# saltoricristiano/lidog

Hardware: AMD Instinct MI355X
Metric: LiDAR scans/sec, MinkUNet34+BEV training step @120k pts (higher is better)
Workload: dtype f32

## Files before the change

### lidog_amd/csrc/conv2d.h

```cpp
#pragma once
#include "common.h"

typedef float f32x16 __attribute__((ext_vector_type(16)));

#define IG_T 128
#define IG_LD 132

struct IgParams {
    const float *A;
    const float *Bm;
    float *D;
    int Bn, Cin, H, W, Cout, Ho, Wo;
    int Mi, Nj, Kd;
    int py, px, nky, nkx, Hc, Wc;
    int ky0, kystep, kx0, kxstep;
    int k_chunk;
};

enum { IG_FWD = 0, IG_DGRAD = 1, IG_WGRAD = 2 };

struct IgClasses {
    IgParams c[4];
    int first[5];
    int n;
    int row_tiles[4];
    long long list_off[4];
};

#define C2_KB 32

void lidog_launch_repack_dgrad_all(const float *W, int Cin, int Cout, float *Wd, hipStream_t st);
```

### lidog_amd/csrc/conv2d.hip

```cpp
#include "common.h"
#include "clock_stamp.h"

#include "conv2d.h"

#define WG_KB 32
#define WG_LD 129
__global__ __launch_bounds__(256) void k_conv_wgrad(IgParams p) {
    __shared__ float As[WG_KB * WG_LD];
    __shared__ float Bs[WG_KB * WG_LD];
    const int tid = threadIdx.x, lane = tid & 63, wave = tid >> 6;
    const int i0 = blockIdx.y * IG_T, j0 = blockIdx.x * IG_T;
    const int HoWo = p.Ho * p.Wo, HW = p.H * p.W;
    const int k_begin = blockIdx.z * p.k_chunk;
    const int k_end = k_begin + p.k_chunk < p.Kd ? k_begin + p.k_chunk : p.Kd;
    const int kk = tid & 31, rg = tid >> 5;

    int cpk[16];
    unsigned a_mask = 0;
#pragma unroll
    for (int r = 0; r < 16; ++r) {
        int j = j0 + rg + 8 * r;
        cpk[r] = -1;
        if (j < p.Nj) {
            int ci = j / 9, t = j - ci * 9;
// ... 76 lines not shown
        load_stage();
        float af[2], bf[2], an[2], bn[2];
        af[0] = a_rd[0]; af[1] = a_rd[32];
        bf[0] = b_rd[0]; bf[1] = b_rd[32];
#pragma unroll
        for (int k2 = 0; k2 < WG_KB / 2; ++k2) {
            if (k2 + 1 < WG_KB / 2) {
                an[0] = a_rd[(2 * k2 + 2) * WG_LD]; an[1] = a_rd[(2 * k2 + 2) * WG_LD + 32];
                bn[0] = b_rd[(2 * k2 + 2) * WG_LD]; bn[1] = b_rd[(2 * k2 + 2) * WG_LD + 32];
            }
            __builtin_amdgcn_sched_barrier(0);
            acc[0][0] = __builtin_amdgcn_mfma_f32_32x32x2f32(af[0], bf[0], acc[0][0], 0, 0, 0);
            acc[0][1] = __builtin_amdgcn_mfma_f32_32x32x2f32(af[0], bf[1], acc[0][1], 0, 0, 0);
            acc[1][0] = __builtin_amdgcn_mfma_f32_32x32x2f32(af[1], bf[0], acc[1][0], 0, 0, 0);
            acc[1][1] = __builtin_amdgcn_mfma_f32_32x32x2f32(af[1], bf[1], acc[1][1], 0, 0, 0);
            __builtin_amdgcn_sched_barrier(0);
            if (k2 + 1 < WG_KB / 2) {
                af[0] = an[0]; af[1] = an[1];
                bf[0] = bn[0]; bf[1] = bn[1];
            }
        }
    }

#pragma unroll
    for (int tj = 0; tj < 2; ++tj) {
        int j = j0 + wj + 32 * tj + li;
        if (j >= p.Nj) continue;
        float *d = p.D + (size_t)blockIdx.z * p.Mi * p.Nj + j;
#pragma unroll
        for (int ti = 0; ti < 2; ++ti) {
#pragma unroll
            for (int e = 0; e < 16; ++e) {
                int i = i0 + wi + 32 * ti + (e & 3) + 8 * (e >> 2) + 4 * kh;
                if (i < p.Mi) d[(size_t)i * p.Nj] = acc[ti][tj][e];
            }
        }
    }
}

template <int MODE, int WM, int TI, int TJ>
__device__ __forceinline__ void conv_s2_tile(const IgParams &p, const int bx, const int by, float *__restrict__ As,
                                             float *__restrict__ Bs) {
    constexpr int TMR = WM * TI * 32;
    constexpr int AV = (TMR * C2_KB / 4) / 256;
    static_assert((4 / WM) * TJ * 32 == IG_T, "tile is 128 pixels wide");
    static_assert((TMR * C2_KB / 4) % 256 == 0, "A stage must divide over the threads");
    extern __shared__ int2 s_tab[];
    const int tid = threadIdx.x, lane = tid & 63, wave = tid >> 6;
    const int i0 = by * TMR, j0 = bx * IG_T;
    const int HoWo = p.Ho * p.Wo, HW = p.H * p.W;
    const int kw = __builtin_amdgcn_readfirstlane(tid >> 7);
    const int nt = p.nky * p.nkx;

    for (int kk = tid; kk < p.Kd; kk += 256) {
        int koff, t;
        if (MODE == IG_FWD) {
            int ci = kk / 9;
            t = kk - ci * 9;
            int ty = t / 3, tx = t - ty * 3;
            koff = ci * HW + (ty - 1) * p.W + (tx - 1);
        } else {
            int co = kk / nt, tap = kk - co * nt;
            int ty = tap / p.nkx, tx = tap - ty * p.nkx;
            koff = co * HoWo - ty * p.Wo - tx;
            t = ty * 2 + tx;
        }
        s_tab[kk] = make_int2(koff, t);
    }

    const int j = j0 + (tid & 127);
    const bool jvalid = j < p.Nj;
    const int jj = jvalid ? j : 0;
    int base, safe;
    unsigned tapmask = 0;
    if (MODE == IG_FWD) {
        int pb = jj / HoWo, r = jj - pb * HoWo;
        int yo = r / p.Wo, xo = r - yo * p.Wo;
        base = pb * p.Cin * HW + (2 * yo) * p.W + 2 * xo;
        safe = base;
#pragma unroll
        for (int ty = 0; ty < 3; ++ty)
#pragma unroll
            for (int tx = 0; tx < 3; ++tx) {
                int y = 2 * yo - 1 + ty, x = 2 * xo - 1 + tx;
                tapmask |= (unsigned)(y >= 0 && y < p.H && x >= 0 && x < p.W) << (ty * 3 + tx);
            }
    } else {
        int hw = p.Hc * p.Wc;
        int pb = jj / hw, r = jj - pb * hw;
        int pyy = (r / p.Wc) * 2 + p.py, pxx = (r % p.Wc) * 2 + p.px;
        int y0 = (pyy + 1 - p.ky0) >> 1, x0 = (pxx + 1 - p.kx0) >> 1;
        safe = pb * p.Cout * HoWo;
        base = safe + y0 * p.Wo + x0;
#pragma unroll
        for (int ty = 0; ty < 2; ++ty)
#pragma unroll
            for (int tx = 0; tx < 2; ++tx)
                tapmask |= (unsigned)(y0 - ty >= 0 && y0 - ty < p.Ho && x0 - tx >= 0 && x0 - tx < p.Wo)
                           << (ty * 2 + tx);
    }
    if (!jvalid) tapmask = 0;

    const float *a_ptr[AV];
    bool a_ok[AV];
#pragma unroll
    for (int v = 0; v < AV; ++v) {
        int f = tid + 256 * v;
        int i = i0 + (f >> 3);
        a_ok[v] = i < p.Mi;
        a_ptr[v] = p.A + (size_t)(a_ok[v] ? i : p.Mi - 1) * p.Kd + (f & 7) * 4;
    }
    __syncthreads();

    float4 ra[AV];
    float rb[16];
    unsigned okbits = 0;
    auto load_stage = [&](int k0) {
#pragma unroll
        for (int v = 0; v < AV; ++v) ra[v] = *reinterpret_cast<const float4 *>(a_ptr[v] + k0);
        okbits = 0;
#pragma unroll
        for (int r = 0; r < 16; ++r) {
            const int2 e = s_tab[k0 + kw + 2 * r];
            const unsigned ok = (tapmask >> e.y) & 1u;
            okbits |= ok << r;
            rb[r] = p.Bm[ok ? base + e.x : safe];
        }
    };
    auto store_stage = [&]() {
#pragma unroll
        for (int v = 0; v < AV; ++v) {
            int f = tid + 256 * v;
            int il = f >> 3, q = f & 7;
            const bool ok = a_ok[v];
            As[(q * 4 + 0) * IG_LD + il] = ok ? ra[v].x : 0.f;
            As[(q * 4 + 1) * IG_LD + il] = ok ? ra[v].y : 0.f;
            As[(q * 4 + 2) * IG_LD + il] = ok ? ra[v].z : 0.f;
            As[(q * 4 + 3) * IG_LD + il] = ok ? ra[v].w : 0.f;
        }
#pragma unroll
        for (int r = 0; r < 16; ++r) Bs[(kw + 2 * r) * IG_LD + (tid & 127)] = ((okbits >> r) & 1u) ? rb[r] : 0.f;
    };

    f32x16 acc[TI][TJ];
#pragma unroll
    for (int a = 0; a < TI; ++a)
#pragma unroll
        for (int b = 0; b < TJ; ++b)
#pragma unroll
            for (int e = 0; e < 16; ++e) acc[a][b][e] = 0.f;
    const int wi = (WM == 1 ? 0 : (wave >> 1)) * (TI * 32), wj = (WM == 1 ? wave : (wave & 1)) * (TJ * 32);
    const int li = lane & 31, kh = lane >> 5;
    const float *a_rd = &As[kh * IG_LD + wi + li];
    const float *b_rd = &Bs[kh * IG_LD + wj + li];

    load_stage(0);
    for (int k0 = 0; k0 < p.Kd; k0 += C2_KB) {
        __syncthreads();
        store_stage();
        __syncthreads();
        load_stage(k0 + C2_KB < p.Kd ? k0 + C2_KB : k0);
        float af[TI], bf[TJ], an[TI], bn[TJ];
#pragma unroll
        for (int a = 0; a < TI; ++a) af[a] = a_rd[32 * a];
#pragma unroll
        for (int b = 0; b < TJ; ++b) bf[b] = b_rd[32 * b];
#pragma unroll
        for (int k2 = 0; k2 < C2_KB / 2; ++k2) {
            if (k2 + 1 < C2_KB / 2) {
#pragma unroll
                for (int a = 0; a < TI; ++a) an[a] = a_rd[(2 * k2 + 2) * IG_LD + 32 * a];
#pragma unroll
                for (int b = 0; b < TJ; ++b) bn[b] = b_rd[(2 * k2 + 2) * IG_LD + 32 * b];
            }
            __builtin_amdgcn_sched_barrier(0);
#pragma unroll
            for (int a = 0; a < TI; ++a)
#pragma unroll
                for (int b = 0; b < TJ; ++b)
                    acc[a][b] = __builtin_amdgcn_mfma_f32_32x32x2f32(af[a], bf[b], acc[a][b], 0, 0, 0);
            __builtin_amdgcn_sched_barrier(0);
            if (k2 + 1 < C2_KB / 2) {
#pragma unroll
                for (int a = 0; a < TI; ++a) af[a] = an[a];
#pragma unroll
                for (int b = 0; b < TJ; ++b) bf[b] = bn[b];
            }
        }
    }

#pragma unroll
    for (int tj = 0; tj < TJ; ++tj) {
        int jo = j0 + wj + 32 * tj + li;
        if (jo >= p.Nj) continue;
        size_t col_off, i_stride;
        if (MODE == IG_FWD) {
            int b = jo / HoWo;
            col_off = (size_t)b * p.Cout * HoWo + (jo - b * HoWo);
            i_stride = HoWo;
        } else {
            int hw = p.Hc * p.Wc;
            int b = jo / hw, r = jo - b * hw;
            int y = (r / p.Wc) * 2 + p.py, x = (r % p.Wc) * 2 + p.px;
            col_off = (size_t)b * p.Cin * HW + (size_t)y * p.W + x;
            i_stride = HW;
        }
#pragma unroll
        for (int ti = 0; ti < TI; ++ti) {
#pragma unroll
            for (int e = 0; e < 16; ++e) {
                int i = i0 + wi + 32 * ti + (e & 3) + 8 * (e >> 2) + 4 * kh;
                if (i < p.Mi) p.D[col_off + (size_t)i * i_stride] = acc[ti][tj][e];
            }
        }
    }
}

template <int MODE, int WM, int TI, int TJ>
__global__ __launch_bounds__(256) void k_conv_s2(IgClasses pc) {
    __shared__ float As[C2_KB * IG_LD];
    __shared__ float Bs[C2_KB * IG_LD];
    const int x = blockIdx.x;
    int cls = 0;
    while (cls + 1 < pc.n && x >= pc.first[cls + 1]) ++cls;
    const IgParams p = pc.c[cls];
    const int r = x - pc.first[cls];
    const int rt = pc.row_tiles[cls];
    LIDOG_STAMP_BEGIN()
    conv_s2_tile<MODE, WM, TI, TJ>(p, r / rt, r % rt, As, Bs);
    LIDOG_STAMP_END()
}

__global__ __launch_bounds__(256) void k_repack_dgrad_all(const float *__restrict__ W, int Cin, int Cout,
                                                          float *__restrict__ Wd) {
    const int64_t cc = (int64_t)Cin * Cout;
    int64_t e = (int64_t)blockIdx.x * 256 + threadIdx.x;
    if (e >= 9 * cc) return;
    const int cls = e < cc ? 0 : e < 3 * cc ? 1 : e < 5 * cc ? 2 : 3;
    const int64_t base = cls == 0 ? 0 : cls == 1 ? cc : cls == 2 ? 3 * cc : 5 * cc;
    const int py = cls >> 1, px = cls & 1;
    const int nky = py ? 2 : 1, nkx = px ? 2 : 1, ky0 = py ? 0 : 1, kx0 = px ? 0 : 1, nt = nky * nkx;
    const int64_t l = e - base;
    int kd = (int)(l % ((int64_t)Cout * nt));
    int ci = (int)(l / ((int64_t)Cout * nt));
    int co = kd / nt, tap = kd % nt;
    int ky = ky0 + (tap / nkx) * 2, kx = kx0 + (tap % nkx) * 2;
    Wd[e] = W[(((size_t)co * Cin + ci) * 3 + ky) * 3 + kx];
}

void lidog_launch_repack_dgrad_all(const float *W, int Cin, int Cout, float *Wd, hipStream_t st) {
    const int64_t total = 9 * (int64_t)Cin * Cout;
    k_repack_dgrad_all<<<(unsigned)cdiv64(total, 256), 256, 0, st>>>(W, Cin, Cout, Wd);
}

__global__ __launch_bounds__(256) void k_sum_splits(const float *__restrict__ partial, int64_t n, int splits,
                                                    int64_t stride, float *__restrict__ out) {
    int64_t i = (int64_t)blockIdx.x * 256 + threadIdx.x;
    if (i >= n) return;
    float acc = partial[i];
    for (int s = 1; s < splits; ++s) acc += partial[(size_t)s * stride + i];
    out[i] = acc;
}

#define PW_MAXCO 8
__global__ __launch_bounds__(256) void k_pw_fwd(const float *__restrict__ X, const float *__restrict__ W,
                                                const float *__restrict__ bias, int Cin, int Cout, int64_t HW,
                                                int64_t total, float *__restrict__ Y) {
    int64_t e = (int64_t)blockIdx.x * 256 + threadIdx.x;
    if (e >= total) return;
    int64_t b = e / HW, pix = e - b * HW;
    float acc[PW_MAXCO];
#pragma unroll
    for (int co = 0; co < PW_MAXCO; ++co) acc[co] = 0.f;
    const float *x = X + (size_t)b * Cin * HW + pix;
// ... 64 lines not shown
            dst[Cout * Cin + co] = (float)(red[PW_MAXCO + co][0] + red[PW_MAXCO + co][1] + red[PW_MAXCO + co][2] +
                                           red[PW_MAXCO + co][3]);
    }
}

static int out_dim(int H, int k, int s, int p) { return (H + 2 * p - k) / s + 1; }

extern "C" int lidog_conv2d_fwd(const float *x, const float *w, const float *bias, int32_t B, int32_t Cin, int32_t H,
                                int32_t W, int32_t Cout, int32_t ksize, int32_t stride, int32_t pad, float *y,
                                void *stream) {
    hipStream_t st = (hipStream_t)stream;
    if (ksize == 1) {
        LIDOG_REQUIRE(stride == 1 && pad == 0 && Cout <= PW_MAXCO, "conv2d_fwd: 1x1 path needs stride 1, Cout <= 8");
        int64_t HW = (int64_t)H * W, total = (int64_t)B * HW;
        if (total) k_pw_fwd<<<(unsigned)cdiv64(total, 256), 256, 0, st>>>(x, w, bias, Cin, Cout, HW, total, y);
        LIDOG_LAUNCH_CHECK();
        return 0;
    }
    LIDOG_REQUIRE(ksize == 3 && stride == 2 && pad == 1 && bias == nullptr,
                  "conv2d_fwd: MFMA path implements k3 s2 p1 without bias (Encoder2D)");
    LIDOG_REQUIRE((Cin * 9) % C2_KB == 0, "conv2d_fwd: Cin*9 must be a multiple of 32");
    IgParams p = {};
    p.A = w; p.Bm = x; p.D = y;
    p.Bn = B; p.Cin = Cin; p.H = H; p.W = W; p.Cout = Cout;
    p.Ho = out_dim(H, 3, 2, 1); p.Wo = out_dim(W, 3, 2, 1);
    p.Mi = Cout; p.Nj = B * p.Ho * p.Wo; p.Kd = Cin * 9;
    if (p.Nj == 0) return 0;
    LIDOG_REQUIRE((int64_t)B * Cin * H * W < ((int64_t)1 << 31) && (int64_t)p.Kd * 8 <= 24576,
                  "conv2d_fwd: tensor too large for 32-bit offsets / reduction table");
    IgClasses pc = {};
    pc.c[0] = p;
    pc.n = 1;
    pc.row_tiles[0] = (int)cdiv64(p.Mi, IG_T);
    pc.first[1] = (int)cdiv64(p.Nj, IG_T) * pc.row_tiles[0];
    k_conv_s2<IG_FWD, 2, 2, 2><<<(unsigned)pc.first[pc.n], 256, (size_t)p.Kd * sizeof(int2), st>>>(pc);
    LIDOG_LAUNCH_CHECK();
    return 0;
}

extern "C" int lidog_conv2d_dgrad(const float *gy, const float *w, int32_t B, int32_t Cin, int32_t H, int32_t W,
                                  int32_t Cout, int32_t ksize, int32_t stride, int32_t pad, float *gx, float *ws,
                                  void *stream) {
    hipStream_t st = (hipStream_t)stream;
    if (ksize == 1) {
        LIDOG_REQUIRE(stride == 1 && pad == 0 && Cout <= PW_MAXCO, "conv2d_dgrad: 1x1 path needs stride 1, Cout <= 8");
        int64_t HW = (int64_t)H * W, total = (int64_t)B * HW;
        if (total) k_pw_dgrad<<<(unsigned)cdiv64(total, 256), 256, 0, st>>>(gy, w, Cin, Cout, HW, total, gx);
        LIDOG_LAUNCH_CHECK();
        return 0;
    }
    LIDOG_REQUIRE(ksize == 3 && stride == 2 && pad == 1, "conv2d_dgrad: MFMA path implements k3 s2 p1");
    LIDOG_REQUIRE(ws != nullptr, "conv2d_dgrad: needs a 9*Cin*Cout float workspace for the repacked weights");
    LIDOG_REQUIRE(Cout % C2_KB == 0, "conv2d_dgrad: Cout must be a multiple of 32");
    LIDOG_REQUIRE((int64_t)B * Cout * out_dim(H, 3, 2, 1) * out_dim(W, 3, 2, 1) < ((int64_t)1 << 31) &&
                      (int64_t)Cout * 4 * 8 <= 24576,
                  "conv2d_dgrad: tensor too large for 32-bit offsets / reduction table");
    int Ho = out_dim(H, 3, 2, 1), Wo = out_dim(W, 3, 2, 1);
    float *slab = ws;
    lidog_launch_repack_dgrad_all(w, Cin, Cout, ws, st);
    const bool rows96 = Cin % 128 != 0 && Cin % 96 == 0;
    IgClasses pc = {};
    IgParams cls_p[4];
    for (int py = 0; py < 2; ++py) {
        for (int px = 0; px < 2; ++px) {
            IgParams &p = cls_p[2 * py + px];
            p = IgParams{};
            p.Bm = gy; p.D = gx;
            p.Bn = B; p.Cin = Cin; p.H = H; p.W = W; p.Cout = Cout; p.Ho = Ho; p.Wo = Wo;
            p.py = py; p.px = px;
            p.nky = py ? 2 : 1; p.ky0 = py ? 0 : 1; p.kystep = 2;
            p.nkx = px ? 2 : 1; p.kx0 = px ? 0 : 1; p.kxstep = 2;
            p.Hc = (H - py + 1) / 2; p.Wc = (W - px + 1) / 2;
            int nt = p.nky * p.nkx;
            p.Mi = Cin; p.Nj = B * p.Hc * p.Wc; p.Kd = Cout * nt;
            int64_t total = (int64_t)Cin * Cout * nt;
            p.A = slab;
            slab += total;
        }
    }
    const int rt = rows96 ? Cin / 96 : (int)cdiv64(Cin, IG_T);
    size_t tab = 0;
    for (int cls : {3, 1, 2, 0}) {
        const IgParams &p = cls_p[cls];
        if (p.Nj <= 0) continue;
        pc.c[pc.n] = p;
        pc.row_tiles[pc.n] = rt;
        pc.first[pc.n + 1] = pc.first[pc.n] + (int)cdiv64(p.Nj, IG_T) * rt;
        ++pc.n;
        if ((size_t)p.Kd * sizeof(int2) > tab) tab = (size_t)p.Kd * sizeof(int2);
    }
    if (pc.n > 0) {
        if (rows96) k_conv_s2<IG_DGRAD, 1, 3, 1><<<(unsigned)pc.first[pc.n], 256, tab, st>>>(pc);
        else k_conv_s2<IG_DGRAD, 2, 2, 2><<<(unsigned)pc.first[pc.n], 256, tab, st>>>(pc);
    }
    LIDOG_LAUNCH_CHECK();
    return 0;
}

extern "C" int lidog_conv2d_wgrad(const float *x, const float *gy, int32_t B, int32_t Cin, int32_t H, int32_t W,
                                  int32_t Cout, int32_t ksize, int32_t stride, int32_t pad, float *gw, float *gbias,
                                  float *ws, int64_t ws_floats, void *stream) {
    hipStream_t st = (hipStream_t)stream;
    if (ksize == 1) {
        LIDOG_REQUIRE(stride == 1 && pad == 0 && Cout <= PW_MAXCO, "conv2d_wgrad: 1x1 path needs stride 1, Cout <= 8");
        const int splits = B * PW_QUARTERS;
        const int64_t slab = (int64_t)Cout * Cin + Cout;
        LIDOG_REQUIRE(ws != nullptr && ws_floats >= splits * slab,
                      "conv2d_wgrad: 1x1 path needs a workspace of %lld floats", (long long)(splits * slab));
        LIDOG_REQUIRE((int64_t)H * W < ((int64_t)1 << 31), "conv2d_wgrad: image too large");
        if (B == 0 || H * W == 0) return 0;
        k_pw_wgrad<<<dim3((unsigned)Cin, (unsigned)splits), 256, 0, st>>>(x, gy, Cin, Cout, H * W, ws);
        k_sum_splits<<<(unsigned)cdiv64((int64_t)Cout * Cin, 256), 256, 0, st>>>(ws, (int64_t)Cout * Cin, splits, slab, gw);
        if (gbias) k_sum_splits<<<1, 256, 0, st>>>(ws + (int64_t)Cout * Cin, Cout, splits, slab, gbias);
        LIDOG_LAUNCH_CHECK();
        return 0;
    }
    LIDOG_REQUIRE(ksize == 3 && stride == 2 && pad == 1 && gbias == nullptr, "conv2d_wgrad: MFMA path implements k3 s2 p1");
    IgParams p = {};
    p.A = gy; p.Bm = x;
    p.Bn = B; p.Cin = Cin; p.H = H; p.W = W; p.Cout = Cout;
    p.Ho = out_dim(H, 3, 2, 1); p.Wo = out_dim(W, 3, 2, 1);
    p.Mi = Cout; p.Nj = Cin * 9; p.Kd = B * p.Ho * p.Wo;
    int64_t slab = (int64_t)p.Mi * p.Nj;
    int tiles = (int)(cdiv64(p.Nj, IG_T) * cdiv64(p.Mi, IG_T));
    int splits = 1024 / tiles;
    if (splits < 1) splits = 1;
    LIDOG_REQUIRE(Cout % 8 == 0, "conv2d_wgrad: Cout must be a multiple of 8");
    LIDOG_REQUIRE((int64_t)Cin * H * W < ((int64_t)1 << 27) && (int64_t)B * Cin * H * W < ((int64_t)1 << 31) &&
                      (int64_t)B * Cout * p.Ho * p.Wo < ((int64_t)1 << 31),
                  "conv2d_wgrad: tensor too large for the packed 32-bit offsets");
    int64_t max_by_k = cdiv64(p.Kd, 4 * WG_KB);
    if (splits > max_by_k) splits = (int)(max_by_k < 1 ? 1 : max_by_k);
    if ((int64_t)splits * slab > ws_floats) splits = (int)(ws_floats / slab);
    LIDOG_REQUIRE(splits >= 1, "conv2d_wgrad: workspace too small (%lld floats needed per split)", (long long)slab);
    p.k_chunk = (int)(cdiv64(cdiv64(p.Kd, splits), WG_KB) * WG_KB);
    splits = (int)cdiv64(p.Kd, p.k_chunk);
    p.D = (splits == 1) ? gw : ws;
    dim3 grid((unsigned)cdiv64(p.Nj, IG_T), (unsigned)cdiv64(p.Mi, IG_T), (unsigned)splits);
    k_conv_wgrad<<<grid, 256, 0, st>>>(p);
    if (splits > 1) k_sum_splits<<<(unsigned)cdiv64(slab, 256), 256, 0, st>>>(ws, slab, splits, slab, gw);
    LIDOG_LAUNCH_CHECK();
    return 0;
}

__global__ __launch_bounds__(256) void k_adam(float *__restrict__ p, const float *__restrict__ g,
                                              float *__restrict__ m, float *__restrict__ v, int64_t n, float lr_bc1,
// ... 29 lines not shown
```

### lidog_amd/csrc/conv2d_sparse.hip

```cpp
#include <vector>

#include "conv2d.h"

__global__ __launch_bounds__(256) void k_support_rowbits(const int32_t *__restrict__ sup, int64_t rows, int W,
                                                         int words, uint64_t *__restrict__ bits) {
    const int64_t row = (int64_t)blockIdx.x * 4 + (threadIdx.x >> 6);
    const int lane = threadIdx.x & 63;
    if (row >= rows) return;
    const int32_t *s = sup + row * W;
    for (int w = 0; w < words; ++w) {
        const int x = w * 64 + lane;
        const bool v = x < W && s[x] >= 0;
        const uint64_t bal = __ballot(v);
        if (lane == 0) bits[row * words + w] = bal;
    }
}

struct ListGeom {
    int C, H, W, Hc, Wc, Nj;
    int ya, ny, xlo, xhi;
    uint64_t mask;
};

__device__ __forceinline__ void tile_list(const uint64_t *__restrict__ bits, int words, const ListGeom &g,
// ... 106 lines not shown
    off += 4 * (int64_t)L.fwd_tiles;
    L.groups = (C + WA_GC - 1) / WA_GC;
    L.glists_off = off;
    off += (int64_t)L.groups * (L.fwd_tiles + 1);
    for (int cls = 0; cls < 4; ++cls) {
        int py = cls >> 1, px = cls & 1;
        int Hc = (H - py + 1) / 2, Wc = (W - px + 1) / 2;
        L.dgrad_tiles[cls] = (int)cdiv64((int64_t)B * Hc * Wc, IG_T);
        L.dgrad_off[cls] = off;
        off += (int64_t)L.dgrad_tiles[cls] * (C + 1);
    }
    L.total = off;
    return L;
}

extern "C" int64_t lidog_conv2d_support_ws(int32_t B, int32_t Cin, int32_t H, int32_t W) {
    return act_layout(B, Cin, H, W).total;
}

extern "C" int lidog_conv2d_support(const int32_t *support, int32_t B, int32_t Cin, int32_t H, int32_t W,
                                    int32_t *act, void *stream) {
    hipStream_t st = (hipStream_t)stream;
    LIDOG_REQUIRE(Cin >= 1 && Cin <= 128, "conv2d_support: 1 <= Cin <= 128");
    LIDOG_REQUIRE((int64_t)B * Cin * H * W < ((int64_t)1 << 31), "conv2d_support: tensor too large");
    if ((int64_t)B * H * W == 0) return 0;
    ActLayout L = act_layout(B, Cin, H, W);
    uint64_t *bits = reinterpret_cast<uint64_t *>(act + L.bits_off);
    int64_t rows = (int64_t)B * Cin * H;
    if (support)
        k_support_rowbits<<<(unsigned)cdiv64(rows, 4), 256, 0, st>>>(support, rows, W, L.words, bits);
    ListGeom g;
    g.C = Cin; g.H = H; g.W = W;
    g.Hc = out_dim2(H); g.Wc = out_dim2(W); g.Nj = B * g.Hc * g.Wc;
    g.ya = -1; g.ny = 3; g.xlo = -1; g.xhi = 1; g.mask = ~0ull;
    uint64_t *tbits = reinterpret_cast<uint64_t *>(act + L.tbits_off);
    k_tile_lists<<<(unsigned)L.fwd_tiles, 128, 0, st>>>(bits, L.words, g, act + L.fwd_off, tbits);
    k_group_lists<<<(unsigned)L.groups, 256, 0, st>>>(tbits, L.fwd_tiles, Cin, act + L.glists_off);
    ListGeom4 q;
    q.first[0] = 0;
    for (int cls = 0; cls < 4; ++cls) {
        int py = cls >> 1, px = cls & 1;
        g.Hc = (H - py + 1) / 2; g.Wc = (W - px + 1) / 2; g.Nj = B * g.Hc * g.Wc;
        g.ya = py; g.ny = 1; g.xlo = px; g.xhi = px;
        g.mask = px ? 0xAAAAAAAAAAAAAAAAull : 0x5555555555555555ull;
        q.g[cls] = g;
        q.off[cls] = L.dgrad_off[cls];
        q.first[cls + 1] = q.first[cls] + L.dgrad_tiles[cls];
    }
    if (q.first[4] > 0) k_tile_lists4<<<(unsigned)q.first[4], 128, 0, st>>>(bits, L.words, q, act);
    LIDOG_LAUNCH_CHECK();
    return 0;
}

__global__ __launch_bounds__(256) void k_conv_fwd_act(IgParams p, const int32_t *__restrict__ lists,
                                                      const float *__restrict__ Wt) {
    __shared__ __attribute__((aligned(16))) float As[C2_KB * IG_LD];
    __shared__ float Bs[C2_KB * IG_LD];
    extern __shared__ int2 s_tab[];
    const int tid = threadIdx.x, lane = tid & 63, wave = tid >> 6;
    const int i0 = blockIdx.y * IG_T, j0 = blockIdx.x * IG_T;
    const int HoWo = p.Ho * p.Wo, HW = p.H * p.W;
    const int kw = __builtin_amdgcn_readfirstlane(tid >> 7);
    const int32_t *lst = lists + (size_t)blockIdx.x * (p.Cin + 1);
    const int n_act = lst[0];
    const int Kd = n_act * 9, Kp = (Kd + C2_KB - 1) / C2_KB * C2_KB;

    for (int kk = tid; kk < Kp; kk += 256) {
        int koff = 0, t = 15, row = 0;
        if (kk < Kd) {
            int a = kk / 9;
            t = kk - a * 9;
            int ci = lst[1 + a];
            int ty = t / 3, tx = t - ty * 3;
            koff = ci * HW + (ty - 1) * p.W + (tx - 1);
            row = ci * 9 + t;
        }
        s_tab[kk] = make_int2(koff, t | (row << 4));
    }

    const int j = j0 + (tid & 127);
    const bool jvalid = j < p.Nj;
    const int jj = jvalid ? j : 0;
    int base;
    unsigned tapmask = 0;
    {
        int pb = jj / HoWo, r = jj - pb * HoWo;
        int yo = r / p.Wo, xo = r - yo * p.Wo;
        base = pb * p.Cin * HW + (2 * yo) * p.W + 2 * xo;
#pragma unroll
        for (int ty = 0; ty < 3; ++ty)
#pragma unroll
            for (int tx = 0; tx < 3; ++tx) {
                int y = 2 * yo - 1 + ty, x = 2 * xo - 1 + tx;
                tapmask |= (unsigned)(y >= 0 && y < p.H && x >= 0 && x < p.W) << (ty * 3 + tx);
            }
    }
    if (!jvalid) tapmask = 0;
    const int safe = base;
    __syncthreads();

    float4 ra[4];
    float rb[16];
    unsigned okbits = 0;
    const int a_kr = tid >> 5, a_c4 = (tid & 31) * 4;
    auto load_stage = [&](int k0) {
#pragma unroll
        for (int v = 0; v < 4; ++v) {
            const int row = s_tab[k0 + a_kr + 8 * v].y >> 4;
            ra[v] = *reinterpret_cast<const float4 *>(Wt + (size_t)row * p.Cout + i0 + a_c4);
        }
        okbits = 0;
#pragma unroll
        for (int r = 0; r < 16; ++r) {
            const int2 e = s_tab[k0 + kw + 2 * r];
            const unsigned ok = (tapmask >> (e.y & 15)) & 1u;
            okbits |= ok << r;
            rb[r] = p.Bm[ok ? base + e.x : safe];
        }
    };
    auto store_stage = [&]() {
#pragma unroll
        for (int v = 0; v < 4; ++v) *reinterpret_cast<float4 *>(&As[(a_kr + 8 * v) * IG_LD + a_c4]) = ra[v];
#pragma unroll
        for (int r = 0; r < 16; ++r) Bs[(kw + 2 * r) * IG_LD + (tid & 127)] = ((okbits >> r) & 1u) ? rb[r] : 0.f;
    };

    f32x16 acc[2][2];
#pragma unroll
    for (int a = 0; a < 2; ++a)
#pragma unroll
        for (int b = 0; b < 2; ++b)
#pragma unroll
            for (int e = 0; e < 16; ++e) acc[a][b][e] = 0.f;
    const int wi = (wave >> 1) * 64, wj = (wave & 1) * 64;
    const int li = lane & 31, kh = lane >> 5;
    const float *a_rd = &As[kh * IG_LD + wi + li];
    const float *b_rd = &Bs[kh * IG_LD + wj + li];

    if (Kp > 0) load_stage(0);
    for (int k0 = 0; k0 < Kp; k0 += C2_KB) {
        __syncthreads();
        store_stage();
        __syncthreads();
        load_stage(k0 + C2_KB < Kp ? k0 + C2_KB : k0);
        float af[2], bf[2], an[2], bn[2];
        af[0] = a_rd[0]; af[1] = a_rd[32];
        bf[0] = b_rd[0]; bf[1] = b_rd[32];
#pragma unroll
        for (int k2 = 0; k2 < C2_KB / 2; ++k2) {
            if (k2 + 1 < C2_KB / 2) {
                an[0] = a_rd[(2 * k2 + 2) * IG_LD]; an[1] = a_rd[(2 * k2 + 2) * IG_LD + 32];
                bn[0] = b_rd[(2 * k2 + 2) * IG_LD]; bn[1] = b_rd[(2 * k2 + 2) * IG_LD + 32];
            }
            __builtin_amdgcn_sched_barrier(0);
            acc[0][0] = __builtin_amdgcn_mfma_f32_32x32x2f32(af[0], bf[0], acc[0][0], 0, 0, 0);
            acc[0][1] = __builtin_amdgcn_mfma_f32_32x32x2f32(af[0], bf[1], acc[0][1], 0, 0, 0);
            acc[1][0] = __builtin_amdgcn_mfma_f32_32x32x2f32(af[1], bf[0], acc[1][0], 0, 0, 0);
            acc[1][1] = __builtin_amdgcn_mfma_f32_32x32x2f32(af[1], bf[1], acc[1][1], 0, 0, 0);
            __builtin_amdgcn_sched_barrier(0);
            if (k2 + 1 < C2_KB / 2) {
                af[0] = an[0]; af[1] = an[1];
                bf[0] = bn[0]; bf[1] = bn[1];
            }
        }
    }

#pragma unroll
    for (int tj = 0; tj < 2; ++tj) {
        int jo = j0 + wj + 32 * tj + li;
        if (jo >= p.Nj) continue;
        int b = jo / HoWo;
        size_t col_off = (size_t)b * p.Cout * HoWo + (jo - b * HoWo);
#pragma unroll
        for (int ti = 0; ti < 2; ++ti) {
#pragma unroll
            for (int e = 0; e < 16; ++e) {
                int i = i0 + wi + 32 * ti + (e & 3) + 8 * (e >> 2) + 4 * kh;
                if (i < p.Mi) p.D[col_off + (size_t)i * HoWo] = acc[ti][tj][e];
            }
        }
    }
}

extern "C" int lidog_conv2d_fwd_sparse(const float *x, const float *w, const int32_t *act, int32_t B, int32_t Cin,
                                       int32_t H, int32_t W, int32_t Cout, float *y, float *ws, void *stream) {
    hipStream_t st = (hipStream_t)stream;
    LIDOG_REQUIRE(Cin >= 1 && Cin <= 128 && Cout % IG_T == 0, "conv2d_fwd_sparse: Cin <= 128, Cout a multiple of 128");
    LIDOG_REQUIRE(ws != nullptr, "conv2d_fwd_sparse: needs a Cin*9*Cout float workspace (transposed weights)");
    IgParams p = {};
    p.Bm = x; p.D = y;
    p.Bn = B; p.Cin = Cin; p.H = H; p.W = W; p.Cout = Cout;
    p.Ho = out_dim2(H); p.Wo = out_dim2(W);
    p.Mi = Cout; p.Nj = B * p.Ho * p.Wo; p.Kd = Cin * 9;
    if (p.Nj == 0) return 0;
    LIDOG_REQUIRE((int64_t)B * Cin * H * W < ((int64_t)1 << 31) && (int64_t)(p.Kd + C2_KB) * 8 <= 24576,
                  "conv2d_fwd_sparse: tensor too large for 32-bit offsets / reduction table");
    ActLayout L = act_layout(B, Cin, H, W);
    int rc = lidog_transpose_kernel(w, 1, Cout, p.Kd, ws, stream);
    if (rc) return rc;
    dim3 grid((unsigned)L.fwd_tiles, (unsigned)(Cout / IG_T), 1);
    k_conv_fwd_act<<<grid, 256, (size_t)(p.Kd + C2_KB) * sizeof(int2), st>>>(p, act + L.fwd_off, ws);
    LIDOG_LAUNCH_CHECK();
    return 0;
}

template <int TIA>
__device__ __forceinline__ void conv_dgrad_act_body(const IgParams &p, const int tile, const int *s_ch, int n_act,
                                                    float *As, float *Bs, const int2 *s_tab) {
    const int tid = threadIdx.x, lane = tid & 63, wave = tid >> 6;
    const int j0 = tile * IG_T;
    const int HoWo = p.Ho * p.Wo, HW = p.H * p.W;
    const int kw = __builtin_amdgcn_readfirstlane(tid >> 7);

    const int j = j0 + (tid & 127);
    const bool jvalid = j < p.Nj;
    const int jj = jvalid ? j : 0;
    int base, safe;
    unsigned tapmask = 0;
    {
        int hw = p.Hc * p.Wc;
        int pb = jj / hw, r = jj - pb * hw;
        int pyy = (r / p.Wc) * 2 + p.py, pxx = (r % p.Wc) * 2 + p.px;
        int y0 = (pyy + 1 - p.ky0) >> 1, x0 = (pxx + 1 - p.kx0) >> 1;
        safe = pb * p.Cout * HoWo;
        base = safe + y0 * p.Wo + x0;
#pragma unroll
        for (int ty = 0; ty < 2; ++ty)
#pragma unroll
            for (int tx = 0; tx < 2; ++tx)
                tapmask |= (unsigned)(y0 - ty >= 0 && y0 - ty < p.Ho && x0 - tx >= 0 && x0 - tx < p.Wo)
                           << (ty * 2 + tx);
    }
    if (!jvalid) tapmask = 0;

    const float *a_ptr[TIA];
    bool a_ok[TIA];
#pragma unroll
    for (int v = 0; v < TIA; ++v) {
        int il = 32 * v + (tid >> 3);
        a_ok[v] = il < n_act;
        a_ptr[v] = p.A + (size_t)(a_ok[v] ? s_ch[il] : 0) * p.Kd + (tid & 7) * 4;
    }

    float4 ra[TIA];
    float rb[16];
    unsigned okbits = 0;
    auto load_stage = [&](int k0) {
#pragma unroll
        for (int v = 0; v < TIA; ++v) ra[v] = *reinterpret_cast<const float4 *>(a_ptr[v] + k0);
        okbits = 0;
#pragma unroll
        for (int r = 0; r < 16; ++r) {
            const int2 e = s_tab[k0 + kw + 2 * r];
            const unsigned ok = (tapmask >> e.y) & 1u;
            okbits |= ok << r;
            rb[r] = p.Bm[ok ? base + e.x : safe];
        }
    };
    auto store_stage = [&]() {
#pragma unroll
        for (int v = 0; v < TIA; ++v) {
            int il = 32 * v + (tid >> 3), q = tid & 7;
            const bool ok = a_ok[v];
            As[(q * 4 + 0) * IG_LD + il] = ok ? ra[v].x : 0.f;
            As[(q * 4 + 1) * IG_LD + il] = ok ? ra[v].y : 0.f;
            As[(q * 4 + 2) * IG_LD + il] = ok ? ra[v].z : 0.f;
            As[(q * 4 + 3) * IG_LD + il] = ok ? ra[v].w : 0.f;
        }
#pragma unroll
        for (int r = 0; r < 16; ++r) Bs[(kw + 2 * r) * IG_LD + (tid & 127)] = ((okbits >> r) & 1u) ? rb[r] : 0.f;
    };

    f32x16 acc[TIA];
#pragma unroll
    for (int a = 0; a < TIA; ++a)
#pragma unroll
        for (int e = 0; e < 16; ++e) acc[a][e] = 0.f;
    const int wj = wave * 32;
    const int li = lane & 31, kh = lane >> 5;
    const float *a_rd = &As[kh * IG_LD + li];
    const float *b_rd = &Bs[kh * IG_LD + wj + li];

    load_stage(0);
    for (int k0 = 0; k0 < p.Kd; k0 += C2_KB) {
        __syncthreads();
        store_stage();
        __syncthreads();
        load_stage(k0 + C2_KB < p.Kd ? k0 + C2_KB : k0);
        float af[TIA], an[TIA], bf, bn = 0.f;
#pragma unroll
        for (int a = 0; a < TIA; ++a) af[a] = a_rd[32 * a];
        bf = b_rd[0];
#pragma unroll
        for (int k2 = 0; k2 < C2_KB / 2; ++k2) {
            if (k2 + 1 < C2_KB / 2) {
#pragma unroll
                for (int a = 0; a < TIA; ++a) an[a] = a_rd[(2 * k2 + 2) * IG_LD + 32 * a];
                bn = b_rd[(2 * k2 + 2) * IG_LD];
            }
            __builtin_amdgcn_sched_barrier(0);
#pragma unroll
            for (int a = 0; a < TIA; ++a) acc[a] = __builtin_amdgcn_mfma_f32_32x32x2f32(af[a], bf, acc[a], 0, 0, 0);
            __builtin_amdgcn_sched_barrier(0);
            if (k2 + 1 < C2_KB / 2) {
#pragma unroll
                for (int a = 0; a < TIA; ++a) af[a] = an[a];
                bf = bn;
            }
        }
    }

    const int jo = j0 + wj + li;
    if (jo < p.Nj) {
        int hw = p.Hc * p.Wc;
        int b = jo / hw, r = jo - b * hw;
        int y = (r / p.Wc) * 2 + p.py, x = (r % p.Wc) * 2 + p.px;
        size_t col_off = (size_t)b * p.Cin * HW + (size_t)y * p.W + x;
#pragma unroll
        for (int ti = 0; ti < TIA; ++ti) {
#pragma unroll
            for (int e = 0; e < 16; ++e) {
                int il = 32 * ti + (e & 3) + 8 * (e >> 2) + 4 * kh;
                if (il < n_act) p.D[col_off + (size_t)s_ch[il] * HW] = acc[ti][e];
            }
        }
    }
}

__global__ __launch_bounds__(256) void k_conv_dgrad_act(IgClasses pc, const int32_t *__restrict__ act) {
    __shared__ float As[C2_KB * IG_LD];
    __shared__ float Bs[C2_KB * IG_LD];
    __shared__ int s_ch[128];
    extern __shared__ int2 s_tab[];
    const int tid = threadIdx.x;
    int cls = 0;
    while (cls + 1 < pc.n && (int)blockIdx.x >= pc.first[cls + 1]) ++cls;
    const IgParams p = pc.c[cls];
    const int tile = (int)blockIdx.x - pc.first[cls];
    const int32_t *lst = act + pc.list_off[cls] + (size_t)tile * (p.Cin + 1);
    const int n_act = lst[0];
    if (n_act == 0) return;
    if (tid < n_act) s_ch[tid] = lst[1 + tid];
    const int nt = p.nky * p.nkx, HoWo = p.Ho * p.Wo;
    for (int kk = tid; kk < p.Kd; kk += 256) {
        int co = kk / nt, tap = kk - co * nt;
        int ty = tap / p.nkx, tx = tap - ty * p.nkx;
        s_tab[kk] = make_int2(co * HoWo - ty * p.Wo - tx, ty * 2 + tx);
    }
    __syncthreads();
    if (n_act <= 32) conv_dgrad_act_body<1>(p, tile, s_ch, n_act, As, Bs, s_tab);
    else if (n_act <= 64) conv_dgrad_act_body<2>(p, tile, s_ch, n_act, As, Bs, s_tab);
    else if (n_act <= 96) conv_dgrad_act_body<3>(p, tile, s_ch, n_act, As, Bs, s_tab);
    else conv_dgrad_act_body<4>(p, tile, s_ch, n_act, As, Bs, s_tab);
}

extern "C" int lidog_conv2d_dgrad_sparse(const float *gy, const float *w, const int32_t *act, int32_t B, int32_t Cin,
                                         int32_t H, int32_t W, int32_t Cout, float *gx, float *ws, void *stream) {
    hipStream_t st = (hipStream_t)stream;
    LIDOG_REQUIRE(Cin >= 1 && Cin <= 128 && Cout % C2_KB == 0, "conv2d_dgrad_sparse: Cin <= 128, Cout % 32 == 0");
    LIDOG_REQUIRE(ws != nullptr, "conv2d_dgrad_sparse: needs a 9*Cin*Cout float workspace for the repacked weights");
    int Ho = out_dim2(H), Wo = out_dim2(W);
    LIDOG_REQUIRE((int64_t)B * Cout * Ho * Wo < ((int64_t)1 << 31) && (int64_t)Cout * 4 * 8 <= 24576 &&
                      (int64_t)B * Cin * H * W < ((int64_t)1 << 31),
                  "conv2d_dgrad_sparse: tensor too large for 32-bit offsets / reduction table");
    ActLayout L = act_layout(B, Cin, H, W);
    float *slab = ws;
    lidog_launch_repack_dgrad_all(w, Cin, Cout, ws, st);
    IgParams cls_p[4];
    for (int cls = 0; cls < 4; ++cls) {
        int py = cls >> 1, px = cls & 1;
        IgParams &p = cls_p[cls];
        p = IgParams{};
        p.Bm = gy; p.D = gx;
        p.Bn = B; p.Cin = Cin; p.H = H; p.W = W; p.Cout = Cout; p.Ho = Ho; p.Wo = Wo;
        p.py = py; p.px = px;
        p.nky = py ? 2 : 1; p.ky0 = py ? 0 : 1; p.kystep = 2;
        p.nkx = px ? 2 : 1; p.kx0 = px ? 0 : 1; p.kxstep = 2;
        p.Hc = (H - py + 1) / 2; p.Wc = (W - px + 1) / 2;
        int nt = p.nky * p.nkx;
        p.Mi = Cin; p.Nj = B * p.Hc * p.Wc; p.Kd = Cout * nt;
        int64_t total = (int64_t)Cin * Cout * nt;
        p.A = slab;
        slab += total;
    }
    IgClasses pc = {};
    size_t tab = 0;
    for (int cls : {3, 1, 2, 0}) {
        const IgParams &p = cls_p[cls];
        if (p.Nj <= 0 || L.dgrad_tiles[cls] <= 0) continue;
        pc.c[pc.n] = p;
        pc.list_off[pc.n] = (long long)L.dgrad_off[cls];
        pc.first[pc.n + 1] = pc.first[pc.n] + (int)L.dgrad_tiles[cls];
        ++pc.n;
        if ((size_t)p.Kd * sizeof(int2) > tab) tab = (size_t)p.Kd * sizeof(int2);
    }
    if (pc.n > 0) k_conv_dgrad_act<<<(unsigned)pc.first[pc.n], 256, tab, st>>>(pc, act);
    LIDOG_LAUNCH_CHECK();
    return 0;
}

#define WA_KB 32
#define WA_TPI 16
#define WA_LDA 129
#define WA_LDB (32 * WA_NT + 1)
__global__ __launch_bounds__(256) void k_conv_wgrad_act(IgParams p, const int32_t *__restrict__ glists, int n_tiles,
                                                        int splits) {
    __shared__ float As[WA_KB * WA_LDA];
    __shared__ float Bs[WA_KB * WA_LDB];
    const int tid = threadIdx.x, lane = tid & 63, wave = tid >> 6;
    const int g = blockIdx.x, i0 = blockIdx.y * IG_T, sp = blockIdx.z;
    const int HoWo = p.Ho * p.Wo, HW = p.H * p.W;
    const int32_t *gl = glists + (size_t)g * (n_tiles + 1);
    const int n_g = gl[0];
    const int t_begin = sp * WA_TPI;
    if (sp > 0 && t_begin >= n_g) return;
    const int t_end = t_begin + WA_TPI < n_g ? t_begin + WA_TPI : n_g;
    const int nq = t_end > t_begin ? 4 * (t_end - t_begin) : 0;
    const int kk = tid & 31, rg = tid >> 5;

    int cpk[4 * WA_NT];
#pragma unroll
    for (int r = 0; r < 4 * WA_NT; ++r) {
        int j = rg + 8 * r;
        int ci = g * WA_GC + j / 9, t = j % 9;
        cpk[r] = -1;
        if (j < 9 * WA_GC && ci < p.Cin) {
            int ty = t / 3, tx = t - ty * 3;
            cpk[r] = ((ci * HW + ty * p.W + tx) << 4) | t;
        }
    }
    unsigned a_mask = 0;
#pragma unroll
    for (int r = 0; r < 16; ++r) a_mask |= (unsigned)(i0 + rg + 8 * r < p.Mi) << r;

    float ra[16], rb[4 * WA_NT];
    unsigned okb = 0;
    bool mv = false;
    const int n_my = t_end - t_begin;
    int tile_cur = n_my > 0 ? gl[1 + t_begin] : 0;
    int tile_nxt = n_my > 1 ? gl[2 + t_begin] : tile_cur;
    auto load_stage = [&](int q) {
        if ((q & 3) == 0 && q > 0) {
            tile_cur = tile_nxt;
            const int ahead = (q >> 2) + 1;
            tile_nxt = gl[1 + t_begin + (ahead < n_my ? ahead : n_my - 1)];
        }
        const int tile = tile_cur;
        const int m = tile * IG_T + (q & 3) * WA_KB + kk;
        mv = m < p.Kd;
// ... 157 lines not shown
```

Baseline: 84.82.

## Replace dgrad tap lookup table with precomputed per-thread offsets and raise occupancy

Result: faster. 85.70, median of 6 (+1.0%).

```diff
diff --git a/lidog_amd/csrc/conv2d.h b/lidog_amd/csrc/conv2d.h
--- a/lidog_amd/csrc/conv2d.h
+++ b/lidog_amd/csrc/conv2d.h
@@ -28,5 +28,9 @@
 };
 
 #define C2_KB 32
+#define C2_LD 129
+#ifndef C2_WAVES
+#define C2_WAVES 3
+#endif
 
 void lidog_launch_repack_dgrad_all(const float *W, int Cin, int Cout, float *Wd, hipStream_t st);
diff --git a/lidog_amd/csrc/conv2d.hip b/lidog_amd/csrc/conv2d.hip
--- a/lidog_amd/csrc/conv2d.hip
+++ b/lidog_amd/csrc/conv2d.hip
@@ -152,20 +152,13 @@
     const int kw = __builtin_amdgcn_readfirstlane(tid >> 7);
     const int nt = p.nky * p.nkx;
 
-    for (int kk = tid; kk < p.Kd; kk += 256) {
-        int koff, t;
-        if (MODE == IG_FWD) {
+    if (MODE == IG_FWD) {
+        for (int kk = tid; kk < p.Kd; kk += 256) {
             int ci = kk / 9;
-            t = kk - ci * 9;
+            int t = kk - ci * 9;
             int ty = t / 3, tx = t - ty * 3;
-            koff = ci * HW + (ty - 1) * p.W + (tx - 1);
-        } else {
-            int co = kk / nt, tap = kk - co * nt;
-            int ty = tap / p.nkx, tx = tap - ty * p.nkx;
-            koff = co * HoWo - ty * p.Wo - tx;
-            t = ty * 2 + tx;
-        }
-        s_tab[kk] = make_int2(koff, t);
+            s_tab[kk] = make_int2(ci * HW + (ty - 1) * p.W + (tx - 1), t);
+        }
     }
 
     const int j = j0 + (tid & 127);
@@ -201,6 +194,20 @@
     }
     if (!jvalid) tapmask = 0;
 
+    int boff[2];
+    unsigned okfix = 0;
+    if (MODE == IG_DGRAD) {
+#pragma unroll
+        for (int s = 0; s < 2; ++s) {
+            const int kr = kw + 2 * s, co = kr / nt, tap = kr - co * nt;
+            const int ty = tap / p.nkx, tx = tap - ty * p.nkx;
+            const bool ok = (tapmask >> (ty * 2 + tx)) & 1u;
+            okfix |= ok ? (0x5555u << s) : 0u;
+            boff[s] = ok ? base + co * HoWo - ty * p.Wo - tx : safe + co * HoWo;
+        }
+    }
+    const int plane4 = (4 / nt) * HoWo;
+
     const float *a_ptr[AV];
     bool a_ok[AV];
 #pragma unroll
@@ -218,13 +225,19 @@
     auto load_stage = [&](int k0) {
 #pragma unroll
         for (int v = 0; v < AV; ++v) ra[v] = *reinterpret_cast<const float4 *>(a_ptr[v] + k0);
-        okbits = 0;
-#pragma unroll
-        for (int r = 0; r < 16; ++r) {
-            const int2 e = s_tab[k0 + kw + 2 * r];
-            const unsigned ok = (tapmask >> e.y) & 1u;
-            okbits |= ok << r;
-            rb[r] = p.Bm[ok ? base + e.x : safe];
+        if (MODE == IG_DGRAD) {
+            const float *bp = p.Bm + (k0 / nt) * HoWo;
+#pragma unroll
+            for (int r = 0; r < 16; ++r) rb[r] = bp[(r >> 1) * plane4 + boff[r & 1]];
+        } else {
+            okbits = 0;
+#pragma unroll
+            for (int r = 0; r < 16; ++r) {
+                const int2 e = s_tab[k0 + kw + 2 * r];
+                const unsigned ok = (tapmask >> e.y) & 1u;
+                okbits |= ok << r;
+                rb[r] = p.Bm[ok ? base + e.x : safe];
+            }
         }
     };
     auto store_stage = [&]() {
@@ -233,13 +246,14 @@
             int f = tid + 256 * v;
             int il = f >> 3, q = f & 7;
             const bool ok = a_ok[v];
-            As[(q * 4 + 0) * IG_LD + il] = ok ? ra[v].x : 0.f;
-            As[(q * 4 + 1) * IG_LD + il] = ok ? ra[v].y : 0.f;
-            As[(q * 4 + 2) * IG_LD + il] = ok ? ra[v].z : 0.f;
-            As[(q * 4 + 3) * IG_LD + il] = ok ? ra[v].w : 0.f;
-        }
-#pragma unroll
-        for (int r = 0; r < 16; ++r) Bs[(kw + 2 * r) * IG_LD + (tid & 127)] = ((okbits >> r) & 1u) ? rb[r] : 0.f;
+            As[(q * 4 + 0) * C2_LD + il] = ok ? ra[v].x : 0.f;
+            As[(q * 4 + 1) * C2_LD + il] = ok ? ra[v].y : 0.f;
+            As[(q * 4 + 2) * C2_LD + il] = ok ? ra[v].z : 0.f;
+            As[(q * 4 + 3) * C2_LD + il] = ok ? ra[v].w : 0.f;
+        }
+        const unsigned okb = MODE == IG_DGRAD ? okfix : okbits;
+#pragma unroll
+        for (int r = 0; r < 16; ++r) Bs[(kw + 2 * r) * C2_LD + (tid & 127)] = ((okb >> r) & 1u) ? rb[r] : 0.f;
     };
 
     f32x16 acc[TI][TJ];
@@ -251,8 +265,8 @@
             for (int e = 0; e < 16; ++e) acc[a][b][e] = 0.f;
     const int wi = (WM == 1 ? 0 : (wave >> 1)) * (TI * 32), wj = (WM == 1 ? wave : (wave & 1)) * (TJ * 32);
     const int li = lane & 31, kh = lane >> 5;
-    const float *a_rd = &As[kh * IG_LD + wi + li];
-    const float *b_rd = &Bs[kh * IG_LD + wj + li];
+    const float *a_rd = &As[kh * C2_LD + wi + li];
+    const float *b_rd = &Bs[kh * C2_LD + wj + li];
 
     load_stage(0);
     for (int k0 = 0; k0 < p.Kd; k0 += C2_KB) {
@@ -269,9 +283,9 @@
         for (int k2 = 0; k2 < C2_KB / 2; ++k2) {
             if (k2 + 1 < C2_KB / 2) {
 #pragma unroll
-                for (int a = 0; a < TI; ++a) an[a] = a_rd[(2 * k2 + 2) * IG_LD + 32 * a];
-#pragma unroll
-                for (int b = 0; b < TJ; ++b) bn[b] = b_rd[(2 * k2 + 2) * IG_LD + 32 * b];
+                for (int a = 0; a < TI; ++a) an[a] = a_rd[(2 * k2 + 2) * C2_LD + 32 * a];
+#pragma unroll
+                for (int b = 0; b < TJ; ++b) bn[b] = b_rd[(2 * k2 + 2) * C2_LD + 32 * b];
             }
             __builtin_amdgcn_sched_barrier(0);
 #pragma unroll
@@ -317,9 +331,9 @@
 }
 
 template <int MODE, int WM, int TI, int TJ>
-__global__ __launch_bounds__(256) void k_conv_s2(IgClasses pc) {
-    __shared__ float As[C2_KB * IG_LD];
-    __shared__ float Bs[C2_KB * IG_LD];
+__global__ __launch_bounds__(256, MODE == IG_FWD ? C2_WAVES : 2) void k_conv_s2(IgClasses pc) {
+    __shared__ float As[C2_KB * C2_LD];
+    __shared__ float Bs[C2_KB * C2_LD];
     const int x = blockIdx.x;
     int cls = 0;
     while (cls + 1 < pc.n && x >= pc.first[cls + 1]) ++cls;
@@ -490,9 +504,8 @@
     LIDOG_REQUIRE(ksize == 3 && stride == 2 && pad == 1, "conv2d_dgrad: MFMA path implements k3 s2 p1");
     LIDOG_REQUIRE(ws != nullptr, "conv2d_dgrad: needs a 9*Cin*Cout float workspace for the repacked weights");
     LIDOG_REQUIRE(Cout % C2_KB == 0, "conv2d_dgrad: Cout must be a multiple of 32");
-    LIDOG_REQUIRE((int64_t)B * Cout * out_dim(H, 3, 2, 1) * out_dim(W, 3, 2, 1) < ((int64_t)1 << 31) &&
-                      (int64_t)Cout * 4 * 8 <= 24576,
-                  "conv2d_dgrad: tensor too large for 32-bit offsets / reduction table");
+    LIDOG_REQUIRE((int64_t)B * Cout * out_dim(H, 3, 2, 1) * out_dim(W, 3, 2, 1) < ((int64_t)1 << 31),
+                  "conv2d_dgrad: tensor too large for 32-bit offsets");
     int Ho = out_dim(H, 3, 2, 1), Wo = out_dim(W, 3, 2, 1);
     float *slab = ws;
     lidog_launch_repack_dgrad_all(w, Cin, Cout, ws, st);
@@ -517,7 +530,6 @@
         }
     }
     const int rt = rows96 ? Cin / 96 : (int)cdiv64(Cin, IG_T);
-    size_t tab = 0;
     for (int cls : {3, 1, 2, 0}) {
         const IgParams &p = cls_p[cls];
         if (p.Nj <= 0) continue;
@@ -525,11 +537,10 @@
         pc.row_tiles[pc.n] = rt;
         pc.first[pc.n + 1] = pc.first[pc.n] + (int)cdiv64(p.Nj, IG_T) * rt;
         ++pc.n;
-        if ((size_t)p.Kd * sizeof(int2) > tab) tab = (size_t)p.Kd * sizeof(int2);
     }
     if (pc.n > 0) {
-        if (rows96) k_conv_s2<IG_DGRAD, 1, 3, 1><<<(unsigned)pc.first[pc.n], 256, tab, st>>>(pc);
-        else k_conv_s2<IG_DGRAD, 2, 2, 2><<<(unsigned)pc.first[pc.n], 256, tab, st>>>(pc);
+        if (rows96) k_conv_s2<IG_DGRAD, 1, 3, 1><<<(unsigned)pc.first[pc.n], 256, 0, st>>>(pc);
+        else k_conv_s2<IG_DGRAD, 2, 2, 2><<<(unsigned)pc.first[pc.n], 256, 0, st>>>(pc);
     }
     LIDOG_LAUNCH_CHECK();
     return 0;
diff --git a/lidog_amd/csrc/conv2d_sparse.hip b/lidog_amd/csrc/conv2d_sparse.hip
--- a/lidog_amd/csrc/conv2d_sparse.hip
+++ b/lidog_amd/csrc/conv2d_sparse.hip
@@ -182,7 +182,7 @@
     return 0;
 }
 
-__global__ __launch_bounds__(256) void k_conv_fwd_act(IgParams p, const int32_t *__restrict__ lists,
+__global__ __launch_bounds__(256, C2_WAVES) void k_conv_fwd_act(IgParams p, const int32_t *__restrict__ lists,
                                                       const float *__restrict__ Wt) {
     __shared__ __attribute__((aligned(16))) float As[C2_KB * IG_LD];
     __shared__ float Bs[C2_KB * IG_LD];
@@ -229,7 +229,8 @@
     const int safe = base;
     __syncthreads();
 
-    float4 ra[4];
+    typedef float f32x4 __attribute__((ext_vector_type(4)));
+    f32x4 ra[4];
     float rb[16];
     unsigned okbits = 0;
     const int a_kr = tid >> 5, a_c4 = (tid & 31) * 4;
@@ -237,7 +238,7 @@
 #pragma unroll
         for (int v = 0; v < 4; ++v) {
             const int row = s_tab[k0 + a_kr + 8 * v].y >> 4;
-            ra[v] = *reinterpret_cast<const float4 *>(Wt + (size_t)row * p.Cout + i0 + a_c4);
+            ra[v] = *reinterpret_cast<const f32x4 *>(Wt + (size_t)row * p.Cout + i0 + a_c4);
         }
         okbits = 0;
 #pragma unroll
@@ -250,7 +251,7 @@
     };
     auto store_stage = [&]() {
 #pragma unroll
-        for (int v = 0; v < 4; ++v) *reinterpret_cast<float4 *>(&As[(a_kr + 8 * v) * IG_LD + a_c4]) = ra[v];
+        for (int v = 0; v < 4; ++v) *reinterpret_cast<f32x4 *>(&As[(a_kr + 8 * v) * IG_LD + a_c4]) = ra[v];
 #pragma unroll
         for (int r = 0; r < 16; ++r) Bs[(kw + 2 * r) * IG_LD + (tid & 127)] = ((okbits >> r) & 1u) ? rb[r] : 0.f;
     };
@@ -336,7 +337,7 @@
 
 template <int TIA>
 __device__ __forceinline__ void conv_dgrad_act_body(const IgParams &p, const int tile, const int *s_ch, int n_act,
-                                                    float *As, float *Bs, const int2 *s_tab) {
+                                                    float *As, float *Bs) {
     const int tid = threadIdx.x, lane = tid & 63, wave = tid >> 6;
     const int j0 = tile * IG_T;
     const int HoWo = p.Ho * p.Wo, HW = p.H * p.W;
@@ -362,6 +363,18 @@
                            << (ty * 2 + tx);
     }
     if (!jvalid) tapmask = 0;
+    const int nt = p.nky * p.nkx;
+    int boff[2];
+    unsigned okfix = 0;
+#pragma unroll
+    for (int s = 0; s < 2; ++s) {
+        const int kr = kw + 2 * s, co = kr / nt, tap = kr - co * nt;
+        const int ty = tap / p.nkx, tx = tap - ty * p.nkx;
+        const bool ok = (tapmask >> (ty * 2 + tx)) & 1u;
+        okfix |= ok ? (0x5555u << s) : 0u;
+        boff[s] = ok ? base + co * HoWo - ty * p.Wo - tx : safe + co * HoWo;
+    }
+    const int plane4 = (4 / nt) * HoWo;
 
     const float *a_ptr[TIA];
     bool a_ok[TIA];
@@ -374,31 +387,25 @@
 
     float4 ra[TIA];
     float rb[16];
-    unsigned okbits = 0;
     auto load_stage = [&](int k0) {
 #pragma unroll
         for (int v = 0; v < TIA; ++v) ra[v] = *reinterpret_cast<const float4 *>(a_ptr[v] + k0);
-        okbits = 0;
-#pragma unroll
-        for (int r = 0; r < 16; ++r) {
-            const int2 e = s_tab[k0 + kw + 2 * r];
-            const unsigned ok = (tapmask >> e.y) & 1u;
-            okbits |= ok << r;
-            rb[r] = p.Bm[ok ? base + e.x : safe];
-        }
+        const float *bp = p.Bm + (k0 / nt) * HoWo;
+#pragma unroll
+        for (int r = 0; r < 16; ++r) rb[r] = bp[(r >> 1) * plane4 + boff[r & 1]];
     };
     auto store_stage = [&]() {
 #pragma unroll
         for (int v = 0; v < TIA; ++v) {
             int il = 32 * v + (tid >> 3), q = tid & 7;
             const bool ok = a_ok[v];
-            As[(q * 4 + 0) * IG_LD + il] = ok ? ra[v].x : 0.f;
-            As[(q * 4 + 1) * IG_LD + il] = ok ? ra[v].y : 0.f;
-            As[(q * 4 + 2) * IG_LD + il] = ok ? ra[v].z : 0.f;
-            As[(q * 4 + 3) * IG_LD + il] = ok ? ra[v].w : 0.f;
-        }
-#pragma unroll
-        for (int r = 0; r < 16; ++r) Bs[(kw + 2 * r) * IG_LD + (tid & 127)] = ((okbits >> r) & 1u) ? rb[r] : 0.f;
+            As[(q * 4 + 0) * C2_LD + il] = ok ? ra[v].x : 0.f;
+            As[(q * 4 + 1) * C2_LD + il] = ok ? ra[v].y : 0.f;
+            As[(q * 4 + 2) * C2_LD + il] = ok ? ra[v].z : 0.f;
+            As[(q * 4 + 3) * C2_LD + il] = ok ? ra[v].w : 0.f;
+        }
+#pragma unroll
+        for (int r = 0; r < 16; ++r) Bs[(kw + 2 * r) * C2_LD + (tid & 127)] = ((okfix >> r) & 1u) ? rb[r] : 0.f;
     };
 
     f32x16 acc[TIA];
@@ -408,8 +415,8 @@
         for (int e = 0; e < 16; ++e) acc[a][e] = 0.f;
     const int wj = wave * 32;
     const int li = lane & 31, kh = lane >> 5;
-    const float *a_rd = &As[kh * IG_LD + li];
-    const float *b_rd = &Bs[kh * IG_LD + wj + li];
+    const float *a_rd = &As[kh * C2_LD + li];
+    const float *b_rd = &Bs[kh * C2_LD + wj + li];
 
     load_stage(0);
     for (int k0 = 0; k0 < p.Kd; k0 += C2_KB) {
@@ -425,8 +432,8 @@
         for (int k2 = 0; k2 < C2_KB / 2; ++k2) {
             if (k2 + 1 < C2_KB / 2) {
 #pragma unroll
-                for (int a = 0; a < TIA; ++a) an[a] = a_rd[(2 * k2 + 2) * IG_LD + 32 * a];
-                bn = b_rd[(2 * k2 + 2) * IG_LD];
+                for (int a = 0; a < TIA; ++a) an[a] = a_rd[(2 * k2 + 2) * C2_LD + 32 * a];
+                bn = b_rd[(2 * k2 + 2) * C2_LD];
             }
             __builtin_amdgcn_sched_barrier(0);
 #pragma unroll
@@ -457,11 +464,10 @@
     }
 }
 
-__global__ __launch_bounds__(256) void k_conv_dgrad_act(IgClasses pc, const int32_t *__restrict__ act) {
-    __shared__ float As[C2_KB * IG_LD];
-    __shared__ float Bs[C2_KB * IG_LD];
+__global__ __launch_bounds__(256, C2_WAVES) void k_conv_dgrad_act(IgClasses pc, const int32_t *__restrict__ act) {
+    __shared__ float As[C2_KB * C2_LD];
+    __shared__ float Bs[C2_KB * C2_LD];
     __shared__ int s_ch[128];
-    extern __shared__ int2 s_tab[];
     const int tid = threadIdx.x;
     int cls = 0;
     while (cls + 1 < pc.n && (int)blockIdx.x >= pc.first[cls + 1]) ++cls;
@@ -471,17 +477,11 @@
     const int n_act = lst[0];
     if (n_act == 0) return;
     if (tid < n_act) s_ch[tid] = lst[1 + tid];
-    const int nt = p.nky * p.nkx, HoWo = p.Ho * p.Wo;
-    for (int kk = tid; kk < p.Kd; kk += 256) {
-        int co = kk / nt, tap = kk - co * nt;
-        int ty = tap / p.nkx, tx = tap - ty * p.nkx;
-        s_tab[kk] = make_int2(co * HoWo - ty * p.Wo - tx, ty * 2 + tx);
-    }
     __syncthreads();
-    if (n_act <= 32) conv_dgrad_act_body<1>(p, tile, s_ch, n_act, As, Bs, s_tab);
-    else if (n_act <= 64) conv_dgrad_act_body<2>(p, tile, s_ch, n_act, As, Bs, s_tab);
-    else if (n_act <= 96) conv_dgrad_act_body<3>(p, tile, s_ch, n_act, As, Bs, s_tab);
-    else conv_dgrad_act_body<4>(p, tile, s_ch, n_act, As, Bs, s_tab);
+    if (n_act <= 32) conv_dgrad_act_body<1>(p, tile, s_ch, n_act, As, Bs);
+    else if (n_act <= 64) conv_dgrad_act_body<2>(p, tile, s_ch, n_act, As, Bs);
+    else if (n_act <= 96) conv_dgrad_act_body<3>(p, tile, s_ch, n_act, As, Bs);
+    else conv_dgrad_act_body<4>(p, tile, s_ch, n_act, As, Bs);
 }
 
 extern "C" int lidog_conv2d_dgrad_sparse(const float *gy, const float *w, const int32_t *act, int32_t B, int32_t Cin,
@@ -490,9 +490,8 @@
     LIDOG_REQUIRE(Cin >= 1 && Cin <= 128 && Cout % C2_KB == 0, "conv2d_dgrad_sparse: Cin <= 128, Cout % 32 == 0");
     LIDOG_REQUIRE(ws != nullptr, "conv2d_dgrad_sparse: needs a 9*Cin*Cout float workspace for the repacked weights");
     int Ho = out_dim2(H), Wo = out_dim2(W);
-    LIDOG_REQUIRE((int64_t)B * Cout * Ho * Wo < ((int64_t)1 << 31) && (int64_t)Cout * 4 * 8 <= 24576 &&
-                      (int64_t)B * Cin * H * W < ((int64_t)1 << 31),
-                  "conv2d_dgrad_sparse: tensor too large for 32-bit offsets / reduction table");
+    LIDOG_REQUIRE((int64_t)B * Cout * Ho * Wo < ((int64_t)1 << 31) && (int64_t)B * Cin * H * W < ((int64_t)1 << 31),
+                  "conv2d_dgrad_sparse: tensor too large for 32-bit offsets");
     ActLayout L = act_layout(B, Cin, H, W);
     float *slab = ws;
     lidog_launch_repack_dgrad_all(w, Cin, Cout, ws, st);
@@ -514,7 +513,6 @@
         slab += total;
     }
     IgClasses pc = {};
-    size_t tab = 0;
     for (int cls : {3, 1, 2, 0}) {
         const IgParams &p = cls_p[cls];
         if (p.Nj <= 0 || L.dgrad_tiles[cls] <= 0) continue;
@@ -522,9 +520,8 @@
         pc.list_off[pc.n] = (long long)L.dgrad_off[cls];
         pc.first[pc.n + 1] = pc.first[pc.n] + (int)L.dgrad_tiles[cls];
         ++pc.n;
-        if ((size_t)p.Kd * sizeof(int2) > tab) tab = (size_t)p.Kd * sizeof(int2);
-    }
-    if (pc.n > 0) k_conv_dgrad_act<<<(unsigned)pc.first[pc.n], 256, tab, st>>>(pc, act);
+    }
+    if (pc.n > 0) k_conv_dgrad_act<<<(unsigned)pc.first[pc.n], 256, 0, st>>>(pc, act);
     LIDOG_LAUNCH_CHECK();
     return 0;
 }
```
